# zhanxw/rvtests

Hardware: AMD Instinct MI355X
Metric: gene-sets/sec (SKAT+SKAT-O+CMC+Zeggini, analytic p-values) (higher is better)
Workload: dtype f64

## Files before the change

rvtests_amd/csrc/k2_unweighted.hip:

```cpp
#include "suffstat_kernels.hip.h"

namespace rvt {

void k2_launch_group_w0(int group, dim3 grid, hipStream_t st, const GeneDesc* d_desc, const int* list, int n_wparts,
                        NullDev nd, long long N, long long ld, int d) {
  const dim3 block(64);
  switch (group) {
    case 0: hipLaunchKernelGGL((gene_suffstat_mfma<0, false>), grid, block, 0, st, d_desc, list, n_wparts, nd, N, ld, d); break;
    case 1: hipLaunchKernelGGL((gene_suffstat_mfma<1, false>), grid, block, 0, st, d_desc, list, n_wparts, nd, N, ld, d); break;
    default: hipLaunchKernelGGL((gene_suffstat_mfma<2, false>), grid, block, 0, st, d_desc, list, n_wparts, nd, N, ld, d); break;
  }
}

void k2_launch_panel_w0(dim3 grid, hipStream_t st, const GeneDesc* d_desc, NullDev nd, long long N, long long ld,
                           int d) {
  hipLaunchKernelGGL((gene_suffstat_panel<false>), grid, dim3(64), 0, st, d_desc, nd, N, ld, d);
}

}
```

rvtests_amd/csrc/k2_weighted.hip:

```cpp
#include "suffstat_kernels.hip.h"

namespace rvt {

void k2_launch_group_w1(int group, dim3 grid, hipStream_t st, const GeneDesc* d_desc, const int* list, int n_wparts,
                        NullDev nd, long long N, long long ld, int d) {
  const dim3 block(64);
  switch (group) {
    case 0: hipLaunchKernelGGL((gene_suffstat_mfma<0, true>), grid, block, 0, st, d_desc, list, n_wparts, nd, N, ld, d); break;
    case 1: hipLaunchKernelGGL((gene_suffstat_mfma<1, true>), grid, block, 0, st, d_desc, list, n_wparts, nd, N, ld, d); break;
    default: hipLaunchKernelGGL((gene_suffstat_mfma<2, true>), grid, block, 0, st, d_desc, list, n_wparts, nd, N, ld, d); break;
  }
}

void k2_launch_panel_w1(dim3 grid, hipStream_t st, const GeneDesc* d_desc, NullDev nd, long long N, long long ld,
                           int d) {
  hipLaunchKernelGGL((gene_suffstat_panel<true>), grid, dim3(64), 0, st, d_desc, nd, N, ld, d);
}

}
```

rvtests_amd/csrc/kernels.hip.h:

```cpp
#pragma once
#include <hip/hip_runtime.h>
#include <float.h>
#include "rvt_pvalue.h"
#include "rvt_mvn.h"

#include "suffstat_kernels.hip.h"
#include "suffstat_hc.hip.h"
#include "suffstat_hcw.hip.h"

namespace rvt {

#if !defined(RVT_K_SPLIT) || defined(RVT_K_ENGINE)
static __global__ __launch_bounds__(64) void gene_flags_kernel(const GeneDesc* __restrict__ genes, long long N) {
  const GeneDesc gd = genes[blockIdx.x];
  if (gd.hc && gd.flags[2 * gd.MT + 1] == 0) return;
  const int tid = threadIdx.x;
  for (int base = 0; base < gd.Mp; base += 64) {
    const int j = base + tid;
    double s = 0.0, mn = INFINITY, mx = -INFINITY;
    if (j < gd.M) {
      for (int p = 0; p < gd.n_wparts; ++p) {
        const double* c = gd.colstat + (long long)p * 3 * gd.Mp;
        s += c[j];
        mn = fmin(mn, c[gd.Mp + j]);
// ... 257 lines not shown
    gd.bparts[(long long)part * 2 * rl + tid] = ((red[0][idx] + red[1][idx]) + red[2][idx]) + red[3][idx];
  }
  __syncthreads();
  }
  }
}

constexpr int kReducePiece = 1024;
#if !defined(RVT_K_SPLIT) || defined(RVT_K_ENGINE)
static __global__ __launch_bounds__(256) void gene_reduce_parts_kernel(const GeneDesc* __restrict__ genes) {
  const GeneDesc gd = genes[blockIdx.y];
  const int Mp = gd.Mp, Cp = gd.Cp, total = Mp * Cp;
  const int idx = blockIdx.x * kReducePiece + (int)threadIdx.x;
  if (blockIdx.x * kReducePiece >= total) return;
  GeneScratch ws = gene_scratch_carve(gd.scratch, Mp, Cp);
  const bool handed_back = gd.hc && gd.flags[2 * gd.MT + 1];
  const double lat_den = (path_integer_gram(gd.hc) && !handed_back) ? gd.lat_den : 0.0;
  const double lat2 = lat_den > 0.0 ? lat_den * lat_den : 0.0;
  const size_t stride = (size_t)Mp * Cp;
  const int P = gd.n_wparts;
  double s4[4];
  bool use[4];
#pragma unroll
  for (int u = 0; u < 4; ++u) {
    const int i = idx + u * 256;
    s4[u] = 0.0;
    use[u] = i < total && ((i % Cp) >> 4) >= ((i / Cp) >> 4);
  }
  for (int p0 = 0; p0 < P; p0 += 8) {
    double t[8][4];
#pragma unroll
    for (int q = 0; q < 8; ++q) {
      const double* src = gd.parts + (size_t)(p0 + q) * stride;
#pragma unroll
      for (int u = 0; u < 4; ++u) t[q][u] = (use[u] && p0 + q < P) ? src[idx + u * 256] : 0.0;
    }
#pragma unroll
    for (int q = 0; q < 8; ++q)
#pragma unroll
      for (int u = 0; u < 4; ++u)
        if (p0 + q < P) s4[u] += t[q][u];
  }
#pragma unroll
  for (int u = 0; u < 4; ++u) {
    const int i = idx + u * 256;
    if (i >= total) continue;
    double sv = s4[u];
    if (use[u] && lat2 > 0.0 && (i % Cp) < gd.M) sv /= lat2;
    ws.R[i] = sv;
  }
}
#endif

#if !defined(RVT_K_SPLIT) || defined(RVT_K_ENGINE)
static __global__ __launch_bounds__(1024) void gene_assemble_kernel(const GeneDesc* __restrict__ genes,
                                                            const NullConsts* __restrict__ ncp, rvt_params prm,
                                                            unsigned tests, int n_bparts, const double* xscale) {
  __shared__ double red[64];
  __shared__ NullConsts nc;
  const GeneDesc gd = genes[blockIdx.x];
  if (threadIdx.x == 0) nc = *ncp;
  __syncthreads();
  Coop co{(int)threadIdx.x, (int)blockDim.x, red};
  GeneScratch ws = gene_scratch_carve(gd.scratch, gd.Mp, gd.Cp);
  const HcMasked hcm{gd.pq, gd.wflags, hc_pq_words(gd.MT), path_integer_gram(gd.hc) ? gd.lat_den : 0.0, gd.pqw, xscale};
  const bool handed_back = gd.hc && gd.flags[2 * gd.MT + 1];
  const bool masks = gd.hc != kPathGeneral && !handed_back;
  gene_assemble(co, nc, gd.M, gd.Mp, gd.Cp, gd.parts, gd.n_wparts, gd.colstat,
                (tests & (RVT_TEST_CMC | RVT_TEST_ZEGGINI)) ? gd.bparts : nullptr, gd.n_bparts > 0 ? gd.n_bparts : n_bparts,
                gd.af, prm, tests, ws,
                gd.stats, gd.dbg_flip, gd.dbg_kept, masks ? &hcm : nullptr, handed_back ? kStatusHandedBack : 0u,
                true);
}
#endif

#if !defined(RVT_K_SPLIT) || defined(RVT_K_ENGINE)
static __global__ __launch_bounds__(256) void gene_tridiag_kernel(const GeneDesc* __restrict__ genes,
                                                           const NullConsts* __restrict__ ncp, unsigned tests,
                                                           int lds_doubles) {
  extern __shared__ __attribute__((aligned(16))) double esm[];
  __shared__ double red[64];
  const GeneDesc gd = genes[blockIdx.y];
  const int which = blockIdx.x;
  Coop co{(int)threadIdx.x, (int)blockDim.x, red};
  GeneScratch ws = gene_scratch_carve(gd.scratch, gd.Mp, gd.Cp);
  const int m = gd.stats->n_poly;
  double* vec = esm;
  double* Bm = (4 * gd.Mp + m * m <= lds_doubles) ? esm + 4 * gd.Mp : ws.eig + (size_t)which * gd.Mp * gd.Mp;
  gene_tridiag(co, *ncp, which, gd.M, gd.Mp, tests, ws, Bm, vec, gd.stats);
}
#endif

#if !defined(RVT_K_SPLIT) || defined(RVT_K_ENGINE)
static __global__ __launch_bounds__(128) void gene_spectrum_kernel(const GeneDesc* __restrict__ genes,
                                                            const NullConsts* __restrict__ ncp, unsigned tests) {
  extern __shared__ __attribute__((aligned(16))) double esm[];
  __shared__ double red[64];
  const GeneDesc gd = genes[blockIdx.y];
  Coop co{(int)threadIdx.x, (int)blockDim.x, red};
  GeneScratch ws = gene_scratch_carve(gd.scratch, gd.Mp, gd.Cp);
  gene_spectrum(co, *ncp, blockIdx.x, gd.M, gd.Mp, tests, ws, esm, gd.stats, gd.lambda);
}
#endif
#if !defined(RVT_K_SPLIT) || defined(RVT_K_ENGINE)
static __global__ __launch_bounds__(128) void gene_spectrum_all_kernel(const GeneDesc* __restrict__ genes,
                                                                const NullConsts* __restrict__ ncp, unsigned tests) {
  extern __shared__ __attribute__((aligned(16))) double esm[];
  __shared__ double red[64];
  __shared__ SpectrumMeta meta[kNEigen];
  const GeneDesc gd = genes[blockIdx.x];
  Coop co{(int)threadIdx.x, (int)blockDim.x, red};
  GeneScratch ws = gene_scratch_carve(gd.scratch, gd.Mp, gd.Cp);
  gene_spectrum_all(co, *ncp, gd.M, gd.Mp, tests, ws, esm, meta, gd.stats, gd.lambda);
}
#endif

struct CovConsts {
  double zzinv[RVT_MAX_COV * RVT_MAX_COV];
  double zsum[RVT_MAX_COV];
  double inv_sigma2;
  double inv_n;
  double c11;
  double k1r;
  double af_denom;
  int d, binary;
  int fam;
};

#if !defined(RVT_K_SPLIT) || defined(RVT_K_ENGINE)
static __global__ __launch_bounds__(256) void cov_prepare_kernel(const GeneDesc* __restrict__ genes, CovConsts cc,
                                                          double* __restrict__ xz, double* __restrict__ colsum,
                                                          int* __restrict__ poly, double* __restrict__ ustat,
                                                          double* __restrict__ afout) {
  const GeneDesc gd = genes[0];
  const int V = gd.M, d = cc.d;
  for (int h = threadIdx.x; h < V; h += blockDim.x) {
    double s = 0.0, mn = INFINITY, mx = -INFINITY;
    for (int p = 0; p < gd.n_wparts; ++p) {
      const double* c = gd.colstat + (long long)p * 3 * gd.Mp;
      s += c[h];
      mn = fmin(mn, c[gd.Mp + h]);
      mx = fmax(mx, c[2 * gd.Mp + h]);
    }
    if (!cc.fam) {
      colsum[h] = s;
      poly[h] = (mn == mx) ? 0 : 1;
    } else {
      s = colsum[h];
      if (ustat) {
        double tu = 0.0, ta = 0.0;
        for (int p = 0; p < gd.n_wparts; ++p) {
          const double* row = gd.parts + (long long)p * gd.Mp * gd.Cp + (long long)h * gd.Cp + V;
          ta += row[d + 1];
          tu += row[d + 2];
        }
        ustat[h] = tu - s * cc.inv_n * cc.k1r;
        afout[h] = (cc.af_denom == 0.0) ? 0.0 : 0.5 * (ta / cc.af_denom);
      }
    }
    for (int k = 0; k < d; ++k) {
      double t = 0.0;
      for (int p = 0; p < gd.n_wparts; ++p)
        t += gd.parts[(long long)p * gd.Mp * gd.Cp + (long long)h * gd.Cp + V + k];
      if (cc.fam)
        xz[(long long)h * d + k] = t - s * cc.inv_n * cc.zsum[k];
      else
// ... 1314 lines not shown
```

rvtests_amd/csrc/rvt_engine.hip:

```cpp
#define RVT_K_SPLIT
#define RVT_K_ENGINE
#include "rvt_engine_int.h"
#include <chrono>
#include <functional>
#include <thread>
#include <sched.h>
#include <sys/syscall.h>
#include <unistd.h>
#include <cctype>

extern "C" {

const char* rvt_version(void) { return "rvtests_amd 0.1 (gfx950)"; }
int64_t rvt_padded_ld(int64_t N) { return (N + 15) / 16 * 16; }
const char* rvt_last_error(const rvt_ctx* ctx) { return ctx ? ctx->err.c_str() : "null context"; }
void* rvt_stream(rvt_ctx* ctx) { return ctx ? (void*)ctx->stream : nullptr; }

int rvt_init(rvt_ctx** out, int device_id) {
  if (!out) return RVT_E_INVALID;
  *out = nullptr;
  int ndev = 0;
  if (hipGetDeviceCount(&ndev) != hipSuccess || ndev <= 0) return RVT_E_NO_DEVICE;
  if (device_id < 0 || device_id >= ndev) return RVT_E_INVALID;
  if (hipSetDevice(device_id) != hipSuccess) return RVT_E_NO_DEVICE;
// ... 82 lines not shown
          hipEventCreateWithFlags(&c->ev_pv_out[i], hipEventDisableTiming);
        }
      } else {
        (void)hipGetLastError();
        for (int k = 0; k < 2; ++k) {
          if (c->pv_stream[k]) hipStreamDestroy(c->pv_stream[k]);
          c->pv_stream[k] = nullptr;
        }
      }
    }
  }
  if (!masked) {
    for (int i = 0; i < kSlots; ++i)
      if (hipStreamCreateWithFlags(&c->slots[i].stream, hipStreamNonBlocking) != hipSuccess) {
        delete c;
        return RVT_E_HIP;
      }
    if (hipStreamCreateWithFlags(&c->k2_stream, hipStreamNonBlocking) != hipSuccess) {
      delete c;
      return RVT_E_HIP;
    }
  }
  if (!c->k2b_stream && hipStreamCreateWithFlags(&c->k2b_stream, hipStreamNonBlocking) != hipSuccess) {
    delete c;
    return RVT_E_HIP;
  }
  c->stream = c->slots[0].stream;
  if (hipStreamCreateWithFlags(&c->io_stream, hipStreamNonBlocking) != hipSuccess ||
      hipStreamCreateWithFlags(&c->copy_stream, hipStreamNonBlocking) != hipSuccess) {
    delete c;
    return RVT_E_HIP;
  }
  c->h2d_stream = c->io_stream;
  for (int k = 0; k < rvt_ctx::kPack; ++k) {
    hipEventCreateWithFlags(&c->ev_pack_copied[k], hipEventDisableTiming);
    hipEventCreateWithFlags(&c->ev_pack_free[k], hipEventDisableTiming);
  }
  for (int i = 0; i < kSlots; ++i) {
    hipEventCreateWithFlags(&c->ev_in[i], hipEventDisableTiming);
    hipEventCreateWithFlags(&c->ev_k2[i], hipEventDisableTiming);
    hipEventCreateWithFlags(&c->ev_k2b[i], hipEventDisableTiming);
  }
  if (c->nc_buf.alloc(sizeof(NullConsts)) != hipSuccess) {
    delete c;
    return RVT_E_HIP;
  }
  c->d_nc = c->nc_buf;
  {
    const int want = 128 * 1024;
    if (hipFuncSetAttribute(reinterpret_cast<const void*>(gene_tridiag_kernel),
                            hipFuncAttributeMaxDynamicSharedMemorySize, want) == hipSuccess)
      c->eigen_lds_max = want;
    (void)hipGetLastError();
  }
  seed_rand_state(c->rand_state, 1u);
  if (const char* e = getenv("RVT_HARDCALL")) c->hc_enabled = atoi(e) != 0;
  if (const char* e = getenv("RVT_STAGE")) c->stage_on = atoi(e) != 0;
  if (const char* e = getenv("RVT_PERM_EXACT")) c->perm_exact = atoi(e) != 0;
  if (const char* e = getenv("RVT_TRACE_SUBMIT")) c->trace_submit = atoi(e) != 0;
  hipEventCreateWithFlags(&c->ev_io, hipEventDisableTiming);
  *out = c;
  return RVT_OK;
}

static void free_null(rvt_ctx* c) {
  c->d_nulltile.reset();
  c->res_buf.reset();
  c->v_buf.reset();
  c->d_X = c->d_res = c->d_rr = c->d_v = c->d_zeros = nullptr;
  c->d_hcp_xq.reset();
  c->d_hcp_scale.reset();
  c->hcp_planes_state = 0;
  c->d_nulltile_w.reset();
  c->d_vq.reset();
  c->d_dq.reset();
  c->d_xq.reset();
  c->d_xscale.reset();
  c->d_fxq.reset();
  c->fdx_ok = false;
  c->hcx_ok = false;
  c->d_null_y.reset();
  c->have_null = false;
}

static void clear_col_kind(rvt_ctx::ColKind& ck) {
  rvt_ctx::ColKind fresh;
  fresh.cols = ck.cols;
  fresh.cache_failed = ck.cache_failed;
  ck = std::move(fresh);
}

void rvt_destroy(rvt_ctx* c) {
  if (!c) return;
  if (c->trace_submit && c->tr_genes > 0)
    fprintf(stderr, "[rvt submit trace] %lld genes: per gene us: total %.1f  copy %.1f  (unused %.1f %.1f)  launch %.1f "
            "| collect total %.1f ms\n", c->tr_genes, 1e6 * c->tr_block / c->tr_genes, 1e6 * c->tr_copy / c->tr_genes,
            1e6 * c->tr_consol / c->tr_genes, 1e6 * c->tr_af / c->tr_genes, 1e6 * c->tr_launch / c->tr_genes,
            1e3 * c->tr_collect);
  hipSetDevice(c->device);
  for (auto& sl : c->slots) sync_stream(sl.stream);
  if (c->io_stream) sync_stream(c->io_stream);
  for (size_t i = 0; i < c->host_reg.size(); ++i)
    if (c->host_reg_owned[i]) (void)hipHostUnregister(const_cast<char*>(c->host_reg[i].first));
  c->host_reg.clear();
  if (c->ev_reg) hipEventDestroy(c->ev_reg);
  if (c->k2b_stream) {
// ... 1214 lines not shown
  }
  return RVT_OK;
}

static int launch_integer_genes(rvt_ctx* c, const Batch& b) {
  const NullConsts& nc = c->nc;
  const long long N = nc.N, ld = nc.ld;
  const int d = nc.d, n = b.n;
  const GeneDesc *h_desc = b.h_desc, *d_desc = b.d_desc;
  const bool hcx = b.caps.hcx;
  static const int planes_sw = getenv("RVT_HCP_PLANES") ? atoi(getenv("RVT_HCP_PLANES")) : 1;
  for (int k = b.n_gen; k < n;) {
    int e = k;
    const int path = h_desc[k].hc, MT = h_desc[k].MT;
    hipStream_t hst = c->k2_stream;
    if (path == kPathHardCall && !hcx && !b.caps.hcw) {
      while (e < n && h_desc[e].hc == path) ++e;
      const int rch = launch_hardcall_classes(c, b, k, e, hst);
      if (rch) return rch;
      k = e;
      continue;
    }
    const bool one_launch = c->hcx_fused && ((hcx && path == kPathHardCall) || path == kPathFloatDigit);
    while (e < n && (one_launch || h_desc[e].MT == MT) && h_desc[e].hc == path && h_desc[e].hcp_planes == h_desc[k].hcp_planes)
      ++e;
    Scope sc(c, 4, hst);
    const dim3 grid(b.n_wparts, e - k);
    const NullTile tile{c->d_nulltile, d + 2};
    if (path == kPathPacked) {
      bool planes = b.caps.nd_is_default && (h_desc[k].hcp_planes || planes_sw == 2) && planes_sw != 0 &&
                    (long long)h_desc[k].steps_per_wpart * 16 <= kHcpPlaneMaxSamples;
      if (planes) {
        const int rcp = ensure_hcp_planes(c);
        if (rcp) return rcp;
        planes = c->hcp_planes_state == 1;
      }
      const HcpPlanes pl{c->d_hcp_xq, c->d_hcp_scale, d + 1};
      k2_launch_hcp(MT, grid, hst, d_desc + k, tile, N, ld, d, planes ? &pl : nullptr,
                    planes && b.cov && b.cov->score && MT <= 2 && !getenv("RVT_SCORE_BED_FULL"));
    } else if (path == kPathFloatDigit)
      k2_launch_fdx(one_launch ? 0 : MT, grid, hst, d_desc + k, c->fdx_tile, N, ld, d);
    else if (path == kPathLattice)
      k2_launch_lat(MT, grid, hst, d_desc + k, tile, (double)c->lattice_den, N, ld, d);
    else if (hcx)
      k2_launch_hcx(one_launch ? 0 : MT, grid, hst, d_desc + k, c->hcx_tile, N, ld, d);
    else
      k2_launch_hcw(MT, grid, hst, d_desc + k, NullTileW{c->d_nulltile_w, d + 3, c->d_vq}, N, ld, d);
    k = e;
  }
  return RVT_OK;
}

static int launch_suffstats(rvt_ctx* c, Batch& b) {
  const int n = b.n, n_gen = b.n_gen, n_hc = b.n_hc, slot_idx = b.slot_idx;
  hipStream_t st = b.st;
  HIP_TRY(c, hipEventRecord(c->ev_in[slot_idx], st));
  HIP_TRY(c, hipStreamWaitEvent(c->k2_stream, c->ev_in[slot_idx], 0));
  const bool split = n_gen > 0 && n_hc > 0 && !b.fdx_batch;
  hipStream_t gst = split ? c->k2b_stream : c->k2_stream;
  if (split) HIP_TRY(c, hipStreamWaitEvent(gst, c->ev_in[slot_idx], 0));
  launch_general_genes(c, b, gst);
  if (b.off.pqw_bytes) HIP_TRY(c, hipMemsetAsync(b.base + b.off.pqw, 0, b.off.pqw_bytes, c->k2_stream));
  int rc = launch_integer_genes(c, b);
  if (rc) return rc;
  if (split) {
    HIP_TRY(c, hipEventRecord(c->ev_k2b[slot_idx], gst));
    HIP_TRY(c, hipStreamWaitEvent(st, c->ev_k2b[slot_idx], 0));
  }
  HIP_TRY(c, hipEventRecord(c->ev_k2[slot_idx], c->k2_stream));
  HIP_TRY(c, hipStreamWaitEvent(st, c->ev_k2[slot_idx], 0));
  if (n_hc > 0) {
    int* d_lists = reinterpret_cast<int*>(b.base + b.off.lists);
    HIP_TRY(c, hipMemsetAsync(d_lists, 0, 4 * sizeof(int), st));
    hipLaunchKernelGGL(gene_flags_hc_kernel, dim3(n_hc), dim3(64), 0, st, b.d_desc + n_gen, (long long)c->nc.N, d_lists, n_hc);
    bool grp_present[3] = {false, false, false};
    for (int k = n_gen; k < n; ++k) grp_present[suffstat_group(b.h_desc[k].MT, b.h_desc[k].CT, c->nc.binary != 0)] = true;
    for (int grp = 0; grp < 3; ++grp)
      if (grp_present[grp]) launch_suffstat(c, st, grp, b.d_desc + n_gen, n_hc, b.n_wparts, b.nd, d_lists);
  }
  b.bt.mark(4);
  return RVT_OK;
}

static int score_tail(rvt_ctx* c, Batch& b) {
  const CovOut* cov = b.cov;
  hipStream_t st = b.st;
  const size_t vt = b.af_total;
  double* d_bur = reinterpret_cast<double*>(b.base + b.off.cov_bur);
  int* d_ok = reinterpret_cast<int*>(b.base + b.off.cov_ok);
  if (cov->wald) {
    WaldConsts wc;
    for (int k = 0; k < RVT_MAX_COV; ++k) wc.beta0[k] = cov->wald_beta0[k];
    hipLaunchKernelGGL(wald_linear_finish_kernel, dim3((unsigned)b.n), dim3(64), 0, st, b.d_desc, c->d_nc, wc, (int)vt, d_bur,
                       d_ok);
  } else {
    hipLaunchKernelGGL(score_finish_kernel, dim3((unsigned)b.n), dim3(64), 0, st, b.d_desc, c->d_nc, (int)vt, d_bur, d_ok);
  }
  HIP_TRY(c, hipGetLastError());
  double* const wald_out[] = {cov->wbeta, cov->wse, cov->wpval};
  double* const score_out[] = {cov->ustat, cov->vstat, cov->effect, cov->se, cov->pval};
  double* const* outs = cov->wald ? wald_out : score_out;
  const int n_out = cov->wald ? 3 : 5;
  const size_t per = cov->wald ? vt * (size_t)c->nc.d : vt;
  for (int k = 0; k < n_out; ++k)
    HIP_TRY(c, hipMemcpyAsync(outs[k], d_bur + k * per, sizeof(double) * per, hipMemcpyDeviceToHost, st));
  HIP_TRY(c, hipMemcpyAsync(cov->ok, d_ok, sizeof(int) * vt, hipMemcpyDeviceToHost, st));
  HIP_TRY(c, sync_stream(st));
  return RVT_OK;
}

static int cov_tail(rvt_ctx* c, Batch& b) {
  const CovOut* cov = b.cov;
  hipStream_t st = b.st;
  char* base = b.base;
  const int V = b.Ms[0];
  CovConsts cc;
  std::vector<double> zz;
  {
    int rcc = cov_constants(c, cov->fam, &cc, &zz);
    if (rcc) return rcc;
    if (cov->fam && cov->uncentred) cc.inv_n = 0.0;
  }
  double* d_xz = reinterpret_cast<double*>(base + b.off.cov_xz);
  double* d_cs = reinterpret_cast<double*>(base + b.off.cov_cs);
  int* d_poly = reinterpret_cast<int*>(base + b.off.cov_poly);
  double* d_cov = reinterpret_cast<double*>(base + b.off.cov);
  if (cov->fam) {
    HIP_TRY(c, hipMemcpyAsync(d_cs, cov->d_raw_colsum, sizeof(double) * (size_t)V, hipMemcpyDeviceToDevice, st));
    HIP_TRY(c, hipMemcpyAsync(d_poly, cov->d_raw_poly, sizeof(int) * (size_t)V, hipMemcpyDeviceToDevice, st));
  }
  double* d_bur = reinterpret_cast<double*>(base + b.off.cov_bur);
// ... 2 lines not shown
                     bur ? d_bur : (double*)nullptr, bur ? d_bur + 2 * (size_t)V : (double*)nullptr);
  hipLaunchKernelGGL(cov_rows_kernel, dim3(V), dim3(256), 0, st, b.d_desc, cc, d_xz, d_cs, d_cov);
  if (bur)
    hipLaunchKernelGGL(fam_burden_finish_kernel, dim3((unsigned)((V + 255) / 256)), dim3(256), 0, st, d_cov, V, d_bur,
                       d_bur + (size_t)V, d_bur + 3 * (size_t)V);
  HIP_TRY(c, hipGetLastError());
  const int dz = cc.d;
  if (cov->cov) HIP_TRY(c, hipMemcpyAsync(cov->cov, d_cov, sizeof(double) * (size_t)V * V, hipMemcpyDeviceToHost, st));
  if (cov->xz) HIP_TRY(c, hipMemcpyAsync(cov->xz, d_xz, sizeof(double) * (size_t)V * dz, hipMemcpyDeviceToHost, st));
  if (cov->poly) HIP_TRY(c, hipMemcpyAsync(cov->poly, d_poly, sizeof(int) * (size_t)V, hipMemcpyDeviceToHost, st));
  if (bur) {
    double* const outs[] = {cov->ustat, cov->vstat, cov->af, cov->pval};
    for (int k = 0; k < 4; ++k)
      HIP_TRY(c, hipMemcpyAsync(outs[k], d_bur + k * (size_t)V, sizeof(double) * (size_t)V, hipMemcpyDeviceToHost, st));
  }
  HIP_TRY(c, sync_stream(st));
  if (cov->zz) std::memcpy(cov->zz, zz.data(), sizeof(double) * (size_t)dz * dz);
  return RVT_OK;
}

static void launch_burden(rvt_ctx* c, const Batch& b) {
  const NullConsts& nc = c->nc;
  const long long N = nc.N, ld = nc.ld;
  const int d = nc.d, n_gen = b.n_gen, n_hc = b.n_hc;
  hipStream_t bs = b.st;
  GeneDesc* d_desc = b.d_desc;
  if (n_gen > 0) {
    {
      Scope sc(c, 1, bs);
      hipLaunchKernelGGL(gene_flags_kernel, dim3(n_gen), dim3(64), 0, bs, d_desc, N);
    }
    const int gpg = 64, ngroups = (n_gen + gpg - 1) / gpg;
    Scope sc(c, 1, bs);
    if (d <= 4)
      hipLaunchKernelGGL((burden_collapse_kernel<4>), dim3(b.n_bparts, ngroups), dim3(256), 0, bs, d_desc, n_gen, gpg, b.nd, N,
                         ld, d, nc.binary, b.tests);
    else
      hipLaunchKernelGGL((burden_collapse_kernel<RVT_MAX_COV>), dim3(b.n_bparts, ngroups), dim3(256), 0, bs, d_desc, n_gen,
                         gpg, b.nd, N, ld, d, nc.binary, b.tests);
  }
  if (n_hc > 0) {
    Scope sc(c, 1, bs);
    const int* d_lists = reinterpret_cast<const int*>(b.base + b.off.lists);
    hipLaunchKernelGGL(gene_flags_kernel, dim3(n_hc), dim3(64), 0, bs, d_desc + n_gen, N);
    if (d <= 4)
      hipLaunchKernelGGL((burden_fallback_kernel<4>), dim3(kFallbackGrid), dim3(256), 0, bs, d_desc + n_gen, d_lists, n_hc,
                         b.n_wparts, b.nd, N, ld, d, nc.binary);
    else
      hipLaunchKernelGGL((burden_fallback_kernel<kHcMaxD>), dim3(kFallbackGrid), dim3(256), 0, bs, d_desc + n_gen, d_lists,
                         n_hc, b.n_wparts, b.nd, N, ld, d, nc.binary);
  }
}

static void launch_assembly(rvt_ctx* c, const Batch& b, unsigned tests_eff) {
  const int n = b.n, d = c->nc.d;
  hipStream_t st = b.st;
  GeneDesc* d_desc = b.d_desc;
  {
    Scope sc(c, 2, st);
    if (b.tests & RVT_TEST_FAMSKAT)
      hipLaunchKernelGGL(fam_assemble_kernel, dim3(n), dim3(1024), 0, st, d_desc, c->d_nc);
    else {
      const int maxMpA = (b.maxM + 15) / 16 * 16, maxCpA = (b.maxM + d + 1 + 15) / 16 * 16;
      hipLaunchKernelGGL(gene_reduce_parts_kernel, dim3((unsigned)((maxMpA * maxCpA + kReducePiece - 1) / kReducePiece), (unsigned)n),
                         dim3(256), 0, st, d_desc);
      hipLaunchKernelGGL(gene_assemble_kernel, dim3(n), dim3(c->as_threads), 0, st, d_desc, c->d_nc, b.params, tests_eff,
                         b.n_bparts, (const double*)c->d_xscale);
    }
  }
  if ((b.tests & RVT_TEST_ANALYTICVT) && !(b.tests & RVT_TEST_FAMSKAT)) {
    Scope sc(c, 2, st);
    hipLaunchKernelGGL(gene_vt_kernel, dim3(n), dim3(256), 0, st, d_desc, c->d_nc);
    for (int stage = 0; stage < 2; ++stage) {
      hipLaunchKernelGGL(vt_integrate_kernel, dim3(n, kMvnShifts), dim3(256), 0, st, d_desc, stage);
      hipLaunchKernelGGL(vt_finish_kernel, dim3((unsigned)((n + 255) / 256)), dim3(256), 0, st, d_desc, n, stage);
    }
  }
}

static void launch_eigen(rvt_ctx* c, const Batch& b, unsigned tests_eig) {
  const int n = b.n, maxM = b.maxM, maxMp = (maxM + 15) / 16 * 16;
  hipStream_t st = b.st;
  GeneDesc* d_desc = b.d_desc;
  {
    Scope sc(c, 2, st);
    size_t want = sizeof(double) * ((size_t)4 * maxMp + (size_t)maxM * maxM);
    if (want > c->eigen_lds_max) want = sizeof(double) * (size_t)4 * maxMp;
    hipLaunchKernelGGL(gene_tridiag_kernel, dim3(kNTridiag, n), dim3(256), want, st, d_desc, c->d_nc, tests_eig,
                       (int)(want / sizeof(double)));
  }
  {
    Scope sc(c, 2, st);
    static const bool per_problem = getenv("RVT_SPECTRUM_PER_PROBLEM") != nullptr;
    const size_t lds_all = sizeof(double) * ((size_t)39 * maxMp + 64);
    if (per_problem || lds_all > ((size_t)60 << 10))
      hipLaunchKernelGGL(gene_spectrum_kernel, dim3(kNEigen, n), dim3(128), sizeof(double) * (size_t)4 * maxMp, st, d_desc,
                         c->d_nc, tests_eig);
    else
      hipLaunchKernelGGL(gene_spectrum_all_kernel, dim3(n), dim3(128), lds_all, st, d_desc, c->d_nc, tests_eig);
  }
}

static int launch_pvalue(rvt_ctx* c, const Batch& b) {
  const int n = b.n, slot_idx = b.slot_idx;
  hipStream_t st = b.st;
  const bool pv_apart = c->pv_cus > 0 && n >= 64 && (b.tests & RVT_TEST_SKATO);
  hipStream_t pst = st;
  if (pv_apart) {
    pst = c->pv_stream[c->pv_turn++ & 1];
    HIP_TRY(c, hipEventRecord(c->ev_pv_in[slot_idx], st));
    HIP_TRY(c, hipStreamWaitEvent(pst, c->ev_pv_in[slot_idx], 0));
  }
  {
    Scope sc(c, 3, pst);
    const size_t smem = sizeof(double) * 4 * ((b.maxM + 1) & ~1) + sizeof(double) * 42 +
                        sizeof(double) * (3 * 64 + 2 * kTermCap) + sizeof(int) * (64 + 64 + 66) + 32;
    if (b.tests & RVT_TEST_EXACT_DAVIES)
      hipLaunchKernelGGL((gene_pvalue_kernel<false>), dim3(n), dim3(64), smem, pst, b.d_desc, b.tests);
    else
      hipLaunchKernelGGL((gene_pvalue_kernel<true>), dim3(n), dim3(64), smem, pst, b.d_desc, b.tests);
  }
  if (pv_apart) {
    HIP_TRY(c, hipEventRecord(c->ev_pv_out[slot_idx], pst));
    HIP_TRY(c, hipStreamWaitEvent(st, c->ev_pv_out[slot_idx], 0));
  }
  return RVT_OK;
}

static int gene_tests_tail(rvt_ctx* c, Batch& b, rvt_gene_result* out) {
  const int n = b.n;
  const uint32_t tests = b.tests;
  Slot& sl = *b.sl;
  const bool burden = (tests & (RVT_TEST_CMC | RVT_TEST_ZEGGINI)) != 0;
  if (burden || b.dbg) launch_burden(c, b);
  const unsigned tests_eff = burden ? tests : (tests & ~(RVT_TEST_CMC | RVT_TEST_ZEGGINI));
  launch_assembly(c, b, tests_eff);
  if (tests & (RVT_TEST_SKAT | RVT_TEST_SKATO | RVT_TEST_FAMSKAT))
    launch_eigen(c, b, (tests & RVT_TEST_FAMSKAT) ? (unsigned)RVT_TEST_SKAT : tests_eff);
  int rc = launch_pvalue(c, b);
  if (rc) return rc;
  HIP_TRY(c, hipGetLastError());
  rvt_gene_result* h_res = reinterpret_cast<rvt_gene_result*>(sl.h_stage + sizeof(GeneDesc) * n +
                                                               (sizeof(double) * b.af_total + 63) / 64 * 64);
  HIP_TRY(c, hipMemcpyAsync(h_res, b.base + b.off.res, sizeof(rvt_gene_result) * n, hipMemcpyDeviceToHost, b.st));
  b.bt.mark(5);
  b.bt.print(n);
  sl.pending_out = out;
  sl.pending_done = c->next_done_flag;
  c->next_done_flag = nullptr;
  sl.h_results = h_res;
  sl.pending_n = n;
  return RVT_OK;
}

static int account_and_inspect(rvt_ctx* c, const Batch& b) {
  const int n = b.n, d = c->nc.d;
  const double N = (double)c->nc.N;
  if (c->profiling) {
    c->timing.genes += n;
    c->timing.genes_hard_call += b.n_hc;
    for (int g = 0; g < n; ++g) {
      const double M = b.Ms[g], null_bytes = 8.0 * N * (d + 2);
      if (b.desc[g].hc == kPathPacked)
        c->timing.alg_bytes_hc += (double)b.desc[g].pk_pitch * M + null_bytes;
      else if (b.desc[g].hc)
        c->timing.alg_bytes_hc += 8.0 * N * M + null_bytes;
      c->timing.alg_bytes += 8.0 * N * M + null_bytes;
      c->timing.alg_flops += 2.0 * N * M * (M + d + 1);
    }
  }
  if (const DebugOut* dbg = b.dbg) {
    HIP_TRY(c, sync_stream(b.st));
    const GeneDesc& g0 = b.desc[0];
    if (dbg->flip) HIP_TRY(c, hipMemcpy(dbg->flip, g0.dbg_flip, sizeof(int) * g0.M, hipMemcpyDeviceToHost));
    if (dbg->kept) HIP_TRY(c, hipMemcpy(dbg->kept, g0.dbg_kept, sizeof(int) * g0.M, hipMemcpyDeviceToHost));
    if (dbg->cmc) HIP_TRY(c, hipMemcpy(dbg->cmc, g0.dbg_cmc, sizeof(double) * c->nc.N, hipMemcpyDeviceToHost));
    if (dbg->zeg) HIP_TRY(c, hipMemcpy(dbg->zeg, g0.dbg_zeg, sizeof(double) * c->nc.N, hipMemcpyDeviceToHost));
    if (dbg->desc0) *dbg->desc0 = g0;
  }
  return RVT_OK;
}

int run_batch(rvt_ctx* c, int n, const double* const* dG, const int* Ms, const double* af,
              const int64_t* ids, uint32_t tests, const rvt_params* prm, rvt_gene_result* out,
              DebugOut* dbg, CovOut* cov, const signed char* kind) {
  Batch b;
  if (!c || n < 0 || (n > 0 && (!dG || !Ms || !af || !out))) return fail(c, RVT_E_INVALID, "bad batch arguments");
  if (!c->have_null) return fail(c, RVT_E_STATE, "no null model set");
  if (n == 0) return RVT_OK;
  hipSetDevice(c->device);
  b.n = n, b.dG = dG, b.Ms = Ms, b.af = af, b.ids = ids, b.tests = tests, b.dbg = dbg, b.cov = cov, b.kind = kind;
// ... 350 lines not shown
```

rvtests_amd/csrc/rvt_engine_int.h:

```cpp
#pragma once
#include <hip/hip_runtime.h>
#include <algorithm>
#include <cstdarg>
#include <cstdio>
#include <cstdlib>
#include <cstring>
#include <ctime>
#include <deque>
#include <map>
#include <string>
#include <unordered_map>
#include <thread>
#include <vector>
#include <cmath>
#include <functional>
#include "kernels.hip.h"
#include "suffstat_lat.hip.h"
#include "suffstat_hcp.hip.h"
#include "suffstat_hcx.hip.h"
#include "suffstat_fdx.hip.h"
#include "host_stage.h"

namespace rvt {
void k2_launch_group_w0(int group, dim3 grid, hipStream_t st, const GeneDesc* d_desc, const int* list, int n_wparts,
// ... 339 lines not shown
  DevBuf<double> d_null_y;
  DevBuf<char> d_wald_ws;
  uint64_t fam_gen = 0;
  double fam_sigma2 = 0.0;
  DevBuf<char> d_lrt_ws;
  uint64_t lrt_gen = 0;
  double lrt_ssr0 = 0.0, lrt_slog = 0.0;
  DevBuf<char> d_gg_ws;
  bool have_grammar = false;
  int64_t gg_N = 0;
  int gg_d = 0;
  double gg_delta = 0.0, gg_gamma = 0.0, gg_ysy = 0.0, gg_sumty = 0.0, gg_afden = 0.0;
  bool have_mt = false;
  int64_t mt_N = 0, mt_ld = 0, mt_ldk = 0;
  int mt_R = 0, mt_K = 0, mt_T = 0;
  size_t mt_plane = 0;
  DevBuf<signed char> d_mt_planes, d_mt_pat, d_mt_B;
  DevBuf<double> d_mt_rowsum;
  DevBuf<char> d_mt_tests, d_mt_ws;
  std::vector<int> mt_row_exp;
  double mt_ms[3] = {0.0, 0.0, 0.0};
  struct Pending {
    int64_t id;
    int M;
    double* dG;
    size_t bytes;
    std::vector<double> af;
    uint32_t tests;
    rvt_params prm;
    rvt_gene_result res;
    bool launched;
    int af_slot = -1;
    int io_error = 0;
    int decoded = 0;
    bool planes = false;
    int kind = kKindUnknown;
  };
  std::deque<Pending> queue;
  std::vector<std::pair<size_t, double*>> block_pool;
  std::vector<std::pair<size_t, double*>> pk_pool;
  struct Launched {
    size_t first;
    int n;
    std::vector<rvt_gene_result> res;
    bool done = false;
  };
  bool* next_done_flag = nullptr;
  std::deque<Launched> launched;
  bool profiling = false;
  std::vector<ProfEvent> events;
  std::vector<hipEvent_t> event_pool;
  rvt_timing timing;
  size_t eigen_lds_max = 48 * 1024;
};

namespace {

int fail(rvt_ctx* c, int code, const char* fmt, ...) {
  if (c) {
    char buf[512];
    va_list ap;
    va_start(ap, fmt);
    vsnprintf(buf, sizeof(buf), fmt, ap);
    va_end(ap);
    c->err = buf;
  }
  return code;
}

#define HIP_TRY(ctx, call)                                                                      \
  do {                                                                                          \
    hipError_t e_ = (call);                                                                     \
    if (e_ != hipSuccess) return fail(ctx, RVT_E_HIP, "%s failed: %s", #call, hipGetErrorString(e_)); \
  } while (0)

int ensure_arena(rvt_ctx* c, Slot& sl, size_t bytes) {
  HIP_TRY(c, sl.arena.grow(bytes, bytes + bytes / 4, sl.stream, true));
  return RVT_OK;
}
int ensure_stage(rvt_ctx* c, Slot& sl, size_t bytes) {
  HIP_TRY(c, sl.h_stage.grow(bytes, bytes * 2, sl.stream));
  return RVT_OK;
}

int finish_slot(rvt_ctx* c, Slot& sl) {
  HIP_TRY(c, sync_stream(sl.stream));
  if (sl.pending_out) {
    bool any_back = false;
    for (int g = 0; g < sl.pending_n; ++g) {
      if (sl.h_results[g].status & kStatusHandedBack) {
        sl.h_results[g].status &= ~kStatusHandedBack;
        any_back = true;
        if (c->profiling) ++c->timing.genes_handed_back;
      }
    }
    if (any_back) c->handed_back_recently = 16;
    else if (c->handed_back_recently > 0) --c->handed_back_recently;
    std::memcpy(sl.pending_out, sl.h_results, sizeof(rvt_gene_result) * sl.pending_n);
    if (sl.pending_done) *sl.pending_done = true;
    sl.pending_done = nullptr;
    sl.pending_out = nullptr;
    sl.pending_n = 0;
  }
  return RVT_OK;
}

// ... 230 lines not shown
```

rvtests_amd/csrc/suffstat_kernels.hip.h:

```cpp
#pragma once
#include <hip/hip_runtime.h>
#include <math.h>
#include "../../include/rvtests_amd.h"

namespace rvt {

struct GeneStats;

enum KernelPath : int {
  kPathGeneral = 0,
  kPathHardCall = 1,
  kPathLattice = 2,
  kPathPacked = 3,
  kPathFloatDigit = 4,
};
__host__ __device__ inline bool path_integer_gram(int hc) { return hc == kPathLattice || hc == kPathFloatDigit; }

typedef double d4_t __attribute__((ext_vector_type(4)));
typedef double d2_t __attribute__((ext_vector_type(2)));
typedef const double __attribute__((address_space(1))) * gcdp_t;
typedef const d2_t __attribute__((address_space(1))) * gcd2p_t;
__device__ __forceinline__ gcdp_t as_global(const double* p) { return (gcdp_t)(unsigned long long)p; }

struct GeneDesc {
// ... 231 lines not shown
    double fg[CT][4];
    const long long sg = full_steps, off = sg * 16 + koff;
    suffstat_load<CT>(colp, off, fg);
    suffstat_step<MT, CT, WEIGHTED, true>(colp, vglob, off, N - off, acc, cs, cmn, cmx, fg, mge + sg * MT * 4,
                                          mle + sg * MT * 4, lane, mask_bytes);
  }
  double* out = gd.parts + (long long)wpart * gd.Mp * gd.Cp;
#pragma unroll
  for (int r = 0; r < MT; ++r) {
#pragma unroll
    for (int c = r; c < CT; ++c) {
#pragma unroll
      for (int i = 0; i < 4; ++i) {
        const int row = r * 16 + (lane >> 4) + 4 * i;
        const int col = c * 16 + (lane & 15);
        out[(long long)row * gd.Cp + col] = acc[r][c][i];
      }
    }
  }
  double* cst = gd.colstat + (long long)wpart * 3 * gd.Mp;
#pragma unroll
  for (int c = 0; c < MT; ++c) {
    double s = cs[c], mn = cmn[c], mx = cmx[c];
    s += __shfl_xor(s, 16, 64);
    mn = fmin(mn, __shfl_xor(mn, 16, 64));
    mx = fmax(mx, __shfl_xor(mx, 16, 64));
    s += __shfl_xor(s, 32, 64);
    mn = fmin(mn, __shfl_xor(mn, 32, 64));
    mx = fmax(mx, __shfl_xor(mx, 32, 64));
    if (lane < 16) {
      cst[c * 16 + lane] = s;
      cst[gd.Mp + c * 16 + lane] = mn;
      cst[2 * gd.Mp + c * 16 + lane] = mx;
    }
  }
}


template <int MT, int CT, bool WEIGHTED>
__device__ __forceinline__ void suffstat_class(const GeneDesc& gd, const NullDev& nd, long long N, long long ld,
                                               int d, int wpart) {
  constexpr int kDepth = (CT <= 3)         ? 3
                         : (MT * CT <= 16) ? (WEIGHTED ? 2 : 3)
                         : (MT * CT <= 20) ? 2
                         : (CT <= 5)       ? 3
                                           : 2;
  suffstat_body<MT, CT, WEIGHTED, kDepth>(gd, nd, N, ld, d, wpart);
}

__host__ __device__ constexpr int suffstat_group(int MT, int CT, bool weighted) {
  return (MT * CT > 20) ? 2 : ((MT * CT <= 4 && !(weighted && MT == 2)) ? 0 : 1);
}

template <int GROUP, bool WEIGHTED>
__global__ __launch_bounds__(64, GROUP == 0 ? 4 : (GROUP == 1 ? 2 : 1)) void gene_suffstat_mfma(
    const GeneDesc* __restrict__ genes, const int* __restrict__ list, int n_wparts, NullDev nd, long long N,
    long long ld, int d) {
  long long item = (long long)blockIdx.x + (long long)blockIdx.y * gridDim.x;
  const long long stride = (long long)gridDim.x * gridDim.y;
  const long long n_items = list ? (long long)list[0] * n_wparts : 0;
  do {
    int gi = blockIdx.y, wpart = blockIdx.x;
    if (list) {
      if (item >= n_items) return;
      gi = list[4 + (int)(item / n_wparts)];
      wpart = (int)(item % n_wparts);
    }
    const GeneDesc gd = genes[gi];
    const int cls = gd.MT * 8 + gd.CT;
#define RVT_CLASS(mt, ct)                                                \
  case mt * 8 + ct:                                                      \
    if constexpr (suffstat_group(mt, ct, WEIGHTED) == GROUP)             \
      suffstat_class<mt, ct, WEIGHTED>(gd, nd, N, ld, d, wpart);         \
    break
    switch (cls) {
      RVT_CLASS(1, 1);
      RVT_CLASS(1, 2);
      RVT_CLASS(2, 2);
      RVT_CLASS(2, 3);
      RVT_CLASS(3, 3);
      RVT_CLASS(3, 4);
      RVT_CLASS(4, 4);
      RVT_CLASS(4, 5);
      RVT_CLASS(5, 5);
      RVT_CLASS(5, 6);
      RVT_CLASS(6, 6);
      RVT_CLASS(6, 7);
      default:
        break;
    }
#undef RVT_CLASS
    item += stride;
  } while (list);
}

template <bool WEIGHTED>
__global__ __launch_bounds__(256) void gene_suffstat_panel(const GeneDesc* __restrict__ genes, NullDev nd, long long N,
                                                           long long ld, int d) {
  const GeneDesc gd = genes[blockIdx.y];
  const int lane = threadIdx.x & 63;
  const int wpart = blockIdx.x * (blockDim.x >> 6) + (threadIdx.x >> 6);
  if (wpart >= gd.n_wparts) return;
  const int nPR = (gd.MT + 3) / 4, nPC = (gd.CT + 3) / 4;
  int pr = 0, pc = 0, z = blockIdx.z;
  for (pr = 0; pr < nPR; ++pr) {
    const int cnt = nPC - pr;
    if (z < cnt) {
      pc = pr + z;
      break;
    }
    z -= cnt;
  }
  if (pr >= nPR) return;
  const bool diag = (pr == pc);
  const int r0 = pr * 4, c0 = pc * 4, M = gd.M, MT = gd.MT;
  const long long nsteps = ld >> 4;
  const long long s_begin = (long long)wpart * gd.steps_per_wpart;
  long long s_end = s_begin + gd.steps_per_wpart;
  if (s_end > nsteps) s_end = nsteps;
  auto column = [&](int j) -> const double* {
    if (j < M) return gd.G + (long long)j * ld;
    if (j < M + d) return nd.X + (long long)(j - M) * ld;
    if (j == M + d) return nd.rr;
    return nd.zeros;
  };
// ... 118 lines not shown
```

Baseline: 26910.

## Fuse assembly, tridiagonalization and spectrum into one LDS-resident per-gene kernel

Adds a gene_dense_kernel that, for genes whose matrices fit in LDS, runs assembly, all tridiagonal reductions and the spectrum step in a single block. It keeps intermediates in shared memory, and the separate kernels early-exit for those genes. This removes several kernel launches and global scratch round-trips per batch. The hard-call suffstat path also launches a single any-group kernel instead of up to three group-specialized launches. In exchange, occupancy is lower from the large LDS footprint and the merged kernel uses a heavier register budget.

```diff
diff --git a/rvtests_amd/csrc/k2_unweighted.hip b/rvtests_amd/csrc/k2_unweighted.hip
--- a/rvtests_amd/csrc/k2_unweighted.hip
+++ b/rvtests_amd/csrc/k2_unweighted.hip
@@ -8,7 +8,8 @@
   switch (group) {
     case 0: hipLaunchKernelGGL((gene_suffstat_mfma<0, false>), grid, block, 0, st, d_desc, list, n_wparts, nd, N, ld, d); break;
     case 1: hipLaunchKernelGGL((gene_suffstat_mfma<1, false>), grid, block, 0, st, d_desc, list, n_wparts, nd, N, ld, d); break;
-    default: hipLaunchKernelGGL((gene_suffstat_mfma<2, false>), grid, block, 0, st, d_desc, list, n_wparts, nd, N, ld, d); break;
+    case 2: hipLaunchKernelGGL((gene_suffstat_mfma<2, false>), grid, block, 0, st, d_desc, list, n_wparts, nd, N, ld, d); break;
+    default: hipLaunchKernelGGL((gene_suffstat_mfma<kSuffstatAnyGroup, false>), grid, block, 0, st, d_desc, list, n_wparts, nd, N, ld, d); break;
   }
 }
 
diff --git a/rvtests_amd/csrc/k2_weighted.hip b/rvtests_amd/csrc/k2_weighted.hip
--- a/rvtests_amd/csrc/k2_weighted.hip
+++ b/rvtests_amd/csrc/k2_weighted.hip
@@ -8,7 +8,8 @@
   switch (group) {
     case 0: hipLaunchKernelGGL((gene_suffstat_mfma<0, true>), grid, block, 0, st, d_desc, list, n_wparts, nd, N, ld, d); break;
     case 1: hipLaunchKernelGGL((gene_suffstat_mfma<1, true>), grid, block, 0, st, d_desc, list, n_wparts, nd, N, ld, d); break;
-    default: hipLaunchKernelGGL((gene_suffstat_mfma<2, true>), grid, block, 0, st, d_desc, list, n_wparts, nd, N, ld, d); break;
+    case 2: hipLaunchKernelGGL((gene_suffstat_mfma<2, true>), grid, block, 0, st, d_desc, list, n_wparts, nd, N, ld, d); break;
+    default: hipLaunchKernelGGL((gene_suffstat_mfma<kSuffstatAnyGroup, true>), grid, block, 0, st, d_desc, list, n_wparts, nd, N, ld, d); break;
   }
 }
 
diff --git a/rvtests_amd/csrc/kernels.hip.h b/rvtests_amd/csrc/kernels.hip.h
--- a/rvtests_amd/csrc/kernels.hip.h
+++ b/rvtests_amd/csrc/kernels.hip.h
@@ -333,13 +333,23 @@
 }
 #endif
 
+constexpr int kDenseThreads = 256;
+constexpr int kDenseIdleTid = (1 << 30) + 1;
+__host__ __device__ constexpr bool gene_dense_fits(int M, int Mp, int lds_doubles) {
+  return 4 * Mp + M * M <= lds_doubles && 39 * Mp + 64 <= lds_doubles;
+}
+__host__ __device__ constexpr int gene_dense_doubles(int M, int Mp) {
+  return 4 * Mp + ((4 * Mp + M * M > 39 * Mp + 64) ? 4 * Mp + M * M : 39 * Mp + 64);
+}
 #if !defined(RVT_K_SPLIT) || defined(RVT_K_ENGINE)
 static __global__ __launch_bounds__(1024) void gene_assemble_kernel(const GeneDesc* __restrict__ genes,
                                                             const NullConsts* __restrict__ ncp, rvt_params prm,
-                                                            unsigned tests, int n_bparts, const double* xscale) {
+                                                            unsigned tests, int n_bparts, const double* xscale,
+                                                            int dense_lds) {
   __shared__ double red[64];
   __shared__ NullConsts nc;
   const GeneDesc gd = genes[blockIdx.x];
+  if (gene_dense_fits(gd.M, gd.Mp, dense_lds)) return;
   if (threadIdx.x == 0) nc = *ncp;
   __syncthreads();
   Coop co{(int)threadIdx.x, (int)blockDim.x, red};
@@ -358,10 +368,11 @@
 #if !defined(RVT_K_SPLIT) || defined(RVT_K_ENGINE)
 static __global__ __launch_bounds__(256) void gene_tridiag_kernel(const GeneDesc* __restrict__ genes,
                                                            const NullConsts* __restrict__ ncp, unsigned tests,
-                                                           int lds_doubles) {
+                                                           int lds_doubles, int dense_lds) {
   extern __shared__ __attribute__((aligned(16))) double esm[];
   __shared__ double red[64];
   const GeneDesc gd = genes[blockIdx.y];
+  if (gene_dense_fits(gd.M, gd.Mp, dense_lds)) return;
   const int which = blockIdx.x;
   Coop co{(int)threadIdx.x, (int)blockDim.x, red};
   GeneScratch ws = gene_scratch_carve(gd.scratch, gd.Mp, gd.Cp);
@@ -374,10 +385,12 @@
 
 #if !defined(RVT_K_SPLIT) || defined(RVT_K_ENGINE)
 static __global__ __launch_bounds__(128) void gene_spectrum_kernel(const GeneDesc* __restrict__ genes,
-                                                            const NullConsts* __restrict__ ncp, unsigned tests) {
+                                                            const NullConsts* __restrict__ ncp, unsigned tests,
+                                                            int dense_lds) {
   extern __shared__ __attribute__((aligned(16))) double esm[];
   __shared__ double red[64];
   const GeneDesc gd = genes[blockIdx.y];
+  if (gene_dense_fits(gd.M, gd.Mp, dense_lds)) return;
   Coop co{(int)threadIdx.x, (int)blockDim.x, red};
   GeneScratch ws = gene_scratch_carve(gd.scratch, gd.Mp, gd.Cp);
   gene_spectrum(co, *ncp, blockIdx.x, gd.M, gd.Mp, tests, ws, esm, gd.stats, gd.lambda);
@@ -385,14 +398,53 @@
 #endif
 #if !defined(RVT_K_SPLIT) || defined(RVT_K_ENGINE)
 static __global__ __launch_bounds__(128) void gene_spectrum_all_kernel(const GeneDesc* __restrict__ genes,
-                                                                const NullConsts* __restrict__ ncp, unsigned tests) {
+                                                                const NullConsts* __restrict__ ncp, unsigned tests,
+                                                                int dense_lds) {
   extern __shared__ __attribute__((aligned(16))) double esm[];
   __shared__ double red[64];
   __shared__ SpectrumMeta meta[kNEigen];
   const GeneDesc gd = genes[blockIdx.x];
+  if (gene_dense_fits(gd.M, gd.Mp, dense_lds)) return;
   Coop co{(int)threadIdx.x, (int)blockDim.x, red};
   GeneScratch ws = gene_scratch_carve(gd.scratch, gd.Mp, gd.Cp);
   gene_spectrum_all(co, *ncp, gd.M, gd.Mp, tests, ws, esm, meta, gd.stats, gd.lambda);
+}
+#endif
+
+#if !defined(RVT_K_SPLIT) || defined(RVT_K_ENGINE)
+static __global__ __launch_bounds__(kDenseThreads) void gene_dense_kernel(const GeneDesc* __restrict__ genes,
+                                                                         const NullConsts* __restrict__ ncp, rvt_params prm,
+                                                                         unsigned tests, int n_bparts, const double* xscale,
+                                                                         int as_threads, int lds_doubles) {
+  extern __shared__ __attribute__((aligned(16))) double esm[];
+  __shared__ double red[64];
+  __shared__ NullConsts nc;
+  __shared__ SpectrumMeta meta[kNEigen];
+  const GeneDesc gd = genes[blockIdx.x];
+  if (!gene_dense_fits(gd.M, gd.Mp, lds_doubles)) return;
+  if (threadIdx.x == 0) nc = *ncp;
+  __syncthreads();
+  const int tid = (int)threadIdx.x;
+  auto coop = [&](int width) { return Coop{tid < width ? tid : kDenseIdleTid, width, red}; };
+  GeneScratch ws = gene_scratch_carve(gd.scratch, gd.Mp, gd.Cp);
+  ws.tri = esm;
+  double* stage = esm + 4 * gd.Mp;
+  {
+    const HcMasked hcm{gd.pq, gd.wflags, hc_pq_words(gd.MT), path_integer_gram(gd.hc) ? gd.lat_den : 0.0, gd.pqw, xscale};
+    const bool handed_back = gd.hc && gd.flags[2 * gd.MT + 1];
+    const bool masks = gd.hc != kPathGeneral && !handed_back;
+    gene_assemble(coop(as_threads), nc, gd.M, gd.Mp, gd.Cp, gd.parts, gd.n_wparts, gd.colstat,
+                  (tests & (RVT_TEST_CMC | RVT_TEST_ZEGGINI)) ? gd.bparts : nullptr, gd.n_bparts > 0 ? gd.n_bparts : n_bparts,
+                  gd.af, prm, tests, ws, gd.stats, gd.dbg_flip, gd.dbg_kept, masks ? &hcm : nullptr,
+                  handed_back ? kStatusHandedBack : 0u, true);
+  }
+  if (!(tests & (RVT_TEST_SKAT | RVT_TEST_SKATO))) return;
+  __syncthreads();
+  for (int which = 0; which < kNTridiag; ++which) {
+    gene_tridiag(coop(256), nc, which, gd.M, gd.Mp, tests, ws, stage + 4 * gd.Mp, stage, gd.stats);
+    __syncthreads();
+  }
+  gene_spectrum_all(coop(128), nc, gd.M, gd.Mp, tests, ws, stage, meta, gd.stats, gd.lambda);
 }
 #endif
 
diff --git a/rvtests_amd/csrc/rvt_engine.hip b/rvtests_amd/csrc/rvt_engine.hip
--- a/rvtests_amd/csrc/rvt_engine.hip
+++ b/rvtests_amd/csrc/rvt_engine.hip
@@ -158,6 +158,14 @@
                             hipFuncAttributeMaxDynamicSharedMemorySize, want) == hipSuccess)
       c->eigen_lds_max = want;
     (void)hipGetLastError();
+  }
+  {
+    const int want = (int)c->eigen_lds_max + 4 * 128 * (int)sizeof(double);
+    if (hipFuncSetAttribute(reinterpret_cast<const void*>(gene_dense_kernel), hipFuncAttributeMaxDynamicSharedMemorySize,
+                            want) == hipSuccess)
+      c->dense_lds_max = want;
+    (void)hipGetLastError();
+    if (const char* e = getenv("RVT_TAIL_FUSED")) c->tail_fused = atoi(e) != 0;
   }
   seed_rand_state(c->rand_state, 1u);
   if (const char* e = getenv("RVT_HARDCALL")) c->hc_enabled = atoi(e) != 0;
@@ -1478,7 +1486,7 @@
 }
 
 static int launch_suffstats(rvt_ctx* c, Batch& b) {
-  const int n = b.n, n_gen = b.n_gen, n_hc = b.n_hc, slot_idx = b.slot_idx;
+  const int n_gen = b.n_gen, n_hc = b.n_hc, slot_idx = b.slot_idx;
   hipStream_t st = b.st;
   HIP_TRY(c, hipEventRecord(c->ev_in[slot_idx], st));
   HIP_TRY(c, hipStreamWaitEvent(c->k2_stream, c->ev_in[slot_idx], 0));
@@ -1499,10 +1507,7 @@
     int* d_lists = reinterpret_cast<int*>(b.base + b.off.lists);
     HIP_TRY(c, hipMemsetAsync(d_lists, 0, 4 * sizeof(int), st));
     hipLaunchKernelGGL(gene_flags_hc_kernel, dim3(n_hc), dim3(64), 0, st, b.d_desc + n_gen, (long long)c->nc.N, d_lists, n_hc);
-    bool grp_present[3] = {false, false, false};
-    for (int k = n_gen; k < n; ++k) grp_present[suffstat_group(b.h_desc[k].MT, b.h_desc[k].CT, c->nc.binary != 0)] = true;
-    for (int grp = 0; grp < 3; ++grp)
-      if (grp_present[grp]) launch_suffstat(c, st, grp, b.d_desc + n_gen, n_hc, b.n_wparts, b.nd, d_lists);
+    launch_suffstat(c, st, kSuffstatAnyGroup, b.d_desc + n_gen, n_hc, b.n_wparts, b.nd, d_lists);
   }
   b.bt.mark(4);
   return RVT_OK;
@@ -1611,7 +1616,31 @@
   }
 }
 
-static void launch_assembly(rvt_ctx* c, const Batch& b, unsigned tests_eff) {
+struct DensePlan {
+  int lds_doubles = 0;
+  size_t lds_bytes = 0;
+  bool all = false;
+};
+static DensePlan plan_dense(const rvt_ctx* c, const Batch& b) {
+  DensePlan p;
+  if (!c->tail_fused || c->as_threads > kDenseThreads || (b.tests & (RVT_TEST_FAMSKAT | RVT_TEST_ANALYTICVT))) return p;
+  const int L = (int)(c->eigen_lds_max / sizeof(double));
+  int taken = 0;
+  for (int g = 0; g < b.n; ++g) {
+    const int M = b.Ms[g], Mp = (M + 15) / 16 * 16;
+    if (!gene_dense_fits(M, Mp, L)) continue;
+    const size_t need = sizeof(double) * (size_t)gene_dense_doubles(M, Mp);
+    if (need > c->dense_lds_max) return DensePlan();
+    p.lds_bytes = std::max(p.lds_bytes, need);
+    ++taken;
+  }
+  if (taken == 0) return DensePlan();
+  p.lds_doubles = L;
+  p.all = taken == b.n;
+  return p;
+}
+
+static void launch_assembly(rvt_ctx* c, const Batch& b, unsigned tests_eff, const DensePlan& dense) {
   const int n = b.n, d = c->nc.d;
   hipStream_t st = b.st;
   GeneDesc* d_desc = b.d_desc;
@@ -1623,8 +1652,12 @@
       const int maxMpA = (b.maxM + 15) / 16 * 16, maxCpA = (b.maxM + d + 1 + 15) / 16 * 16;
       hipLaunchKernelGGL(gene_reduce_parts_kernel, dim3((unsigned)((maxMpA * maxCpA + kReducePiece - 1) / kReducePiece), (unsigned)n),
                          dim3(256), 0, st, d_desc);
-      hipLaunchKernelGGL(gene_assemble_kernel, dim3(n), dim3(c->as_threads), 0, st, d_desc, c->d_nc, b.params, tests_eff,
-                         b.n_bparts, (const double*)c->d_xscale);
+      if (dense.lds_doubles)
+        hipLaunchKernelGGL(gene_dense_kernel, dim3(n), dim3(kDenseThreads), dense.lds_bytes, st, d_desc, c->d_nc, b.params,
+                           tests_eff, b.n_bparts, (const double*)c->d_xscale, c->as_threads, dense.lds_doubles);
+      if (!dense.all)
+        hipLaunchKernelGGL(gene_assemble_kernel, dim3(n), dim3(c->as_threads), 0, st, d_desc, c->d_nc, b.params, tests_eff,
+                           b.n_bparts, (const double*)c->d_xscale, dense.lds_doubles);
     }
   }
   if ((b.tests & RVT_TEST_ANALYTICVT) && !(b.tests & RVT_TEST_FAMSKAT)) {
@@ -1637,7 +1670,8 @@
   }
 }
 
-static void launch_eigen(rvt_ctx* c, const Batch& b, unsigned tests_eig) {
+static void launch_eigen(rvt_ctx* c, const Batch& b, unsigned tests_eig, const DensePlan& dense) {
+  if (dense.all) return;
   const int n = b.n, maxM = b.maxM, maxMp = (maxM + 15) / 16 * 16;
   hipStream_t st = b.st;
   GeneDesc* d_desc = b.d_desc;
@@ -1646,7 +1680,7 @@
     size_t want = sizeof(double) * ((size_t)4 * maxMp + (size_t)maxM * maxM);
     if (want > c->eigen_lds_max) want = sizeof(double) * (size_t)4 * maxMp;
     hipLaunchKernelGGL(gene_tridiag_kernel, dim3(kNTridiag, n), dim3(256), want, st, d_desc, c->d_nc, tests_eig,
-                       (int)(want / sizeof(double)));
+                       (int)(want / sizeof(double)), dense.lds_doubles);
   }
   {
     Scope sc(c, 2, st);
@@ -1654,9 +1688,10 @@
     const size_t lds_all = sizeof(double) * ((size_t)39 * maxMp + 64);
     if (per_problem || lds_all > ((size_t)60 << 10))
       hipLaunchKernelGGL(gene_spectrum_kernel, dim3(kNEigen, n), dim3(128), sizeof(double) * (size_t)4 * maxMp, st, d_desc,
-                         c->d_nc, tests_eig);
+                         c->d_nc, tests_eig, dense.lds_doubles);
     else
-      hipLaunchKernelGGL(gene_spectrum_all_kernel, dim3(n), dim3(128), lds_all, st, d_desc, c->d_nc, tests_eig);
+      hipLaunchKernelGGL(gene_spectrum_all_kernel, dim3(n), dim3(128), lds_all, st, d_desc, c->d_nc, tests_eig,
+                         dense.lds_doubles);
   }
 }
 
@@ -1693,9 +1728,10 @@
   const bool burden = (tests & (RVT_TEST_CMC | RVT_TEST_ZEGGINI)) != 0;
   if (burden || b.dbg) launch_burden(c, b);
   const unsigned tests_eff = burden ? tests : (tests & ~(RVT_TEST_CMC | RVT_TEST_ZEGGINI));
-  launch_assembly(c, b, tests_eff);
+  const DensePlan dense = plan_dense(c, b);
+  launch_assembly(c, b, tests_eff, dense);
   if (tests & (RVT_TEST_SKAT | RVT_TEST_SKATO | RVT_TEST_FAMSKAT))
-    launch_eigen(c, b, (tests & RVT_TEST_FAMSKAT) ? (unsigned)RVT_TEST_SKAT : tests_eff);
+    launch_eigen(c, b, (tests & RVT_TEST_FAMSKAT) ? (unsigned)RVT_TEST_SKAT : tests_eff, dense);
   int rc = launch_pvalue(c, b);
   if (rc) return rc;
   HIP_TRY(c, hipGetLastError());
diff --git a/rvtests_amd/csrc/rvt_engine_int.h b/rvtests_amd/csrc/rvt_engine_int.h
--- a/rvtests_amd/csrc/rvt_engine_int.h
+++ b/rvtests_amd/csrc/rvt_engine_int.h
@@ -415,6 +415,8 @@
   std::vector<hipEvent_t> event_pool;
   rvt_timing timing;
   size_t eigen_lds_max = 48 * 1024;
+  bool tail_fused = true;
+  size_t dense_lds_max = 0;
 };
 
 namespace {
diff --git a/rvtests_amd/csrc/suffstat_kernels.hip.h b/rvtests_amd/csrc/suffstat_kernels.hip.h
--- a/rvtests_amd/csrc/suffstat_kernels.hip.h
+++ b/rvtests_amd/csrc/suffstat_kernels.hip.h
@@ -307,6 +307,7 @@
   return (MT * CT > 20) ? 2 : ((MT * CT <= 4 && !(weighted && MT == 2)) ? 0 : 1);
 }
 
+constexpr int kSuffstatAnyGroup = 3;
 template <int GROUP, bool WEIGHTED>
 __global__ __launch_bounds__(64, GROUP == 0 ? 4 : (GROUP == 1 ? 2 : 1)) void gene_suffstat_mfma(
     const GeneDesc* __restrict__ genes, const int* __restrict__ list, int n_wparts, NullDev nd, long long N,
@@ -325,7 +326,7 @@
     const int cls = gd.MT * 8 + gd.CT;
 #define RVT_CLASS(mt, ct)                                                \
   case mt * 8 + ct:                                                      \
-    if constexpr (suffstat_group(mt, ct, WEIGHTED) == GROUP)             \
+    if constexpr (GROUP == kSuffstatAnyGroup || suffstat_group(mt, ct, WEIGHTED) == GROUP) \
       suffstat_class<mt, ct, WEIGHTED>(gd, nd, N, ld, d, wpart);         \
     break
     switch (cls) {
```

Result: no change. 26850, median of 3 (-0.2%).
